# JensUweUlrich/Taxor

Hardware: AMD Instinct MI355X
Metric: Mbp/s classified (taxor search) vs GTDB k22/s12 (higher is better)
Workload: dtype u8

## Files before the change

taxor_amd/csrc/api.hip:

```cpp
#include "../../include/taxor_gpu_tools.h"
#include "fastx_scan.h"
#include "hip_host.h"
#include "ixf_arith.h"
#include "ixf_layout.h"
#include "kernels.h"
#include "saved_batch.h"
#include "tuning.h"

#include <sys/mman.h>

#include <algorithm>
#include <atomic>
#include <cstdio>
#include <cstring>
#include <mutex>
#include <string>
#include <thread>
#include <vector>

using namespace taxor;

namespace {

thread_local std::string g_err;
// ... 38 lines not shown
    std::mutex plane_mu;
    void *build_ctx = nullptr;
    void (*build_ctx_free)(void *) = nullptr;
    uint32_t n_passes = 0;
    std::vector<uint32_t> pass_of_ixf;
    std::vector<uint64_t> pass_data_bytes;
    uint64_t root_data_bytes = 0;
    uint32_t *d_binfo_full = nullptr;
    uint8_t *d_resident = nullptr;
    int cur_pass = -1;
    int up_group = -1;
    std::thread up_thread;
    int up_rc = 0;
    std::string up_err;
    std::vector<uint8_t> up_select;
    const uint8_t *upload_select = nullptr;
    double upload_wait_s = 0;
    std::mutex searchers_mu;
    std::vector<taxor_gpu_searcher *> searchers;
};

static void root_plane_invalidate(taxor_gpu_index *idx)
{
    std::lock_guard<std::mutex> lk(idx->plane_mu);
    idx->plane_valid = false;
}

static const uint8_t *root_plane_ensure(taxor_gpu_index *idx, hipStream_t st)
{
    if (!idx->plane_stride) return nullptr;
    std::lock_guard<std::mutex> lk(idx->plane_mu);
    if (idx->plane_valid) return idx->d_plane;
    if (!idx->d_plane && hipMalloc((void **)&idx->d_plane, idx->rows[0] * (uint64_t)idx->plane_stride) != hipSuccess) {
        (void)hipGetLastError();
        idx->d_plane = nullptr;
        idx->plane_stride = 0;
        return nullptr;
    }
    launch_build_plane(idx->h_ixf[0].data, idx->rows[0], idx->h_ixf[0].stride, idx->d_plane, idx->plane_stride, st);
    if (hipGetLastError() != hipSuccess || hipStreamSynchronize(st) != hipSuccess) return nullptr;
    idx->plane_valid = true;
    return idx->d_plane;
}

struct SubBatch {
    uint32_t first, n;
    uint32_t n_long = 0;
    uint64_t slots;
    uint64_t a_begin, a_end;
};

struct taxor_gpu_searcher {
    taxor_gpu_index *idx = nullptr;
    taxor_gpu_search_params prm{};
    std::vector<uint32_t> h_rlen, h_nh_sub;
    std::vector<uint64_t> lay_poff, lay_hoff, lay_aoff;
    std::vector<uint32_t> lay_hcap, lay_order;
    std::vector<uint64_t> h_thr_sub;
    bool thr_precomputed = false;
    std::vector<uint64_t> thr_memo;
    hipStream_t st = nullptr;
    hipStream_t st_sync = nullptr;
    hipStream_t st_sync2 = nullptr;
    hipEvent_t ev_wave = nullptr;
    hipStream_t st_copy = nullptr;
    std::vector<hipEvent_t> ev_sync_done, ev_query_done, ev_pack_done, ev_copy_done;
    hipEvent_t ev_reset = nullptr;
    DeviceBuf<uint32_t> d_sync_cursor;
    Counters *d_ctr = nullptr;
    unsigned long long *d_prof = nullptr;
    Counters h_ctr{};
    int grid_query_small[MAX_LEVELS] = {};
    size_t lds_query_small[MAX_LEVELS] = {};
    int grid_wave = 0, grid_wave_overlap = 0;
    int grid_sync = 0, grid_sync_overlap = 0, grid_query = 0, grid_query_short = 0;
    uint32_t first_div = 1;
    bool auto_sub_reads = true;
    bool prune = true;
    bool group_always = false;
    bool split_always = false;
    bool force_tree_stall = false;
    bool small_path = true;
    bool screen = true;
    size_t lds_query = 0;

    struct HostSpan { uint64_t vbegin, len; const char *ptr; };
    std::vector<HostSpan> host_spans;
    uint64_t n_reads = 0, n_bases = 0, mean_read_len = 1u << 20;
    DeviceBuf<uint8_t> d_ascii;
    DeviceBuf<uint64_t> d_aoff, d_poff, d_hoff;
    DeviceBuf<uint32_t> d_packed, d_rlen, d_hcap, d_nh, d_order;
    DeviceBuf<uint64_t> d_thr;
    std::vector<SubBatch> subs;
    uint64_t max_slots = 0, max_read_slots = 0;
    uint32_t max_sub_reads = 0;
    uint64_t packed_word_count = 0, packed_in_bytes = 0;
    FastxScan *fx = nullptr;
    std::vector<uint64_t> fx_off;
    DeviceBuf<uint64_t> d_boff;
    DeviceBuf<uint8_t> d_rev;
    std::vector<uint64_t> nib_off, nib_boff;
    std::vector<uint8_t> nib_rev;
    std::vector<uint32_t> h_words;

    DeviceBuf<uint64_t> d_cand[2], d_hashes[2];
    DeviceBuf<uint2> d_q[2], d_qs;
    DeviceBuf<uint32_t> d_qhist;
    DeviceBuf<uint4> d_hits;
    DeviceBuf<uint32_t> d_read_hits, d_cursor, d_roff, d_biglist, d_gtab, d_scan;
    uint32_t q_cap = 0, hit_cap = 0, gtab_stride = 0;

    DeviceBuf<uint64_t> d_read_off;
    DeviceBuf<int64_t> d_out_ub;
    DeviceBuf<uint32_t> d_out_cnt, d_out_key;
    uint64_t tuple_cap = 0;
    bool ran = false, synced = false;

    std::vector<uint64_t> h_read_off, h_hash_off, h_hashes;
    std::vector<int64_t> h_ub;
    std::vector<uint32_t> h_cnt, h_nh;
    void *h_small = nullptr;
    void *h_small_in = nullptr;

    struct SmallLane {
        taxor_gpu_searcher *c = nullptr;
        hipEvent_t done = nullptr, copied = nullptr;
        DeviceBuf<uint8_t> d_in;
        void *h_in = nullptr;
        size_t h_in_cap = 0;
        void *h_bases = nullptr;
        size_t h_bases_cap = 0;
        void *h_out = nullptr, *d_out = nullptr;
        uint32_t out_reads = 0, out_tuples = 0;
        bool fresh = true;
        bool q_dirty = false;
    };
    struct SmallPiece { uint32_t lane; uint64_t first, n; };
    std::vector<SmallLane> lanes;
    std::vector<SmallPiece> small_pieces;
    const char *small_bases = nullptr;
    const uint64_t *small_offsets = nullptr;
    bool lane_mode = false;
    bool st_borrowed = false;
    bool small_active = false, small_done = false;
    size_t small_harvested = 0;
    uint64_t small_tbase = 0;
    bool dev_results_stale = false;
    bool keep_keys = false;
    std::vector<uint32_t> h_key;

    bool capture = false;
    taxor_gpu_saved *cap_cur = nullptr;
    bool cap_done = false;
    DeviceBuf<uint64_t> d_cap_dense[2], d_cap_off;
    uint64_t *h_cap_pin[2] = {nullptr, nullptr};
    uint64_t *h_cap_total = nullptr;
    hipEvent_t ev_cap[2] = {nullptr, nullptr}, ev_cap_gather[2] = {nullptr, nullptr};
    hipStream_t st_cap = nullptr;
    const taxor_gpu_saved *replay = nullptr;
    bool from_saved = false;

    std::vector<hipEvent_t> ev;
    size_t ev_used = 0;
    std::vector<std::pair<size_t, int>> ev_spans;
    taxor_gpu_run_stats stats{};
};
// ... 753 lines not shown
    if (out) {
        const uint8_t *p = root_plane_ensure(idx, nullptr);
        if (!p) return TAXOR_OK;
        if (len != idx->rows[0] * (uint64_t)idx->plane_stride) return fail(TAXOR_E_ARG, "root_plane: the buffer does not match the plane");
        HIP_TRY(hipMemcpy(out, p, len, hipMemcpyDeviceToHost));
    }
    *rows = idx->rows[0];
    *plane_stride = idx->plane_stride;
    return TAXOR_OK;
}

extern "C" int taxor_gpu_index_download_ixf(const taxor_gpu_index *idx, uint64_t ixf, uint8_t *data, uint64_t len)
{
    if (!idx || ixf >= idx->h_ixf.size() || !data || len != idx->rows[ixf] * idx->h_ixf[ixf].stride)
        return fail(TAXOR_E_ARG, "download_ixf: bad arguments");
    HIP_TRY(hipSetDevice(idx->device));
    HIP_TRY(hipMemcpy(data, idx->h_ixf[ixf].data, len, hipMemcpyDeviceToHost));
    return TAXOR_OK;
}

static int searcher_create_impl(taxor_gpu_index *idx, const taxor_gpu_search_params *prm, taxor_gpu_searcher **out, hipStream_t lane_stream);

extern "C" int taxor_gpu_searcher_create(taxor_gpu_index *idx, const taxor_gpu_search_params *prm,
                                         taxor_gpu_searcher **out)
{
    return searcher_create_impl(idx, prm, out, nullptr);
}

static int searcher_create_impl(taxor_gpu_index *idx, const taxor_gpu_search_params *prm, taxor_gpu_searcher **out, hipStream_t lane_stream)
{
    if (!idx || !prm || !out) return fail(TAXOR_E_ARG, "searcher_create: null argument");
    const bool by_ratio = prm->model == TAXOR_THR_PERCENTAGE || prm->model == TAXOR_THR_SYNCMER;
    if (by_ratio && (!(prm->ratio >= 0.0) || !(prm->ratio <= 1.0)))
        return fail(TAXOR_E_ARG, "searcher_create: threshold ratio %g outside [0,1] (error rate / k outside the model?)", prm->ratio);
    if (prm->model > TAXOR_THR_FRACMINHASH) return fail(TAXOR_E_ARG, "searcher_create: unknown threshold model %u", prm->model);
    if (!by_ratio && (!(prm->error_rate > 0.0) || !(prm->error_rate < 1.0)))
        return fail(TAXOR_E_ARG, "searcher_create: the k-mer / FracMinHash threshold models need an error rate in (0,1), got %g", prm->error_rate);
    if (prm->model == TAXOR_THR_SYNCMER && idx->w_min > 0)
        return fail(TAXOR_E_ARG, "searcher_create: syncmer threshold model on an index built without syncmers");
    HIP_TRY(hipSetDevice(idx->device));
    auto s = new taxor_gpu_searcher();
    s->idx = idx;
    s->prm = *prm;
    s->auto_sub_reads = s->prm.sub_batch_reads == 0;
    if (s->prm.sub_batch_reads == 0) s->prm.sub_batch_reads = 32768;
    if (s->prm.sub_batch_bases == 0) s->prm.sub_batch_bases = 1ull << 29;
    if (s->prm.sub_batch_reads > (1u << 20)) s->prm.sub_batch_reads = 1u << 20;
    hipError_t e = hipSuccess;
    if (lane_stream) {
        s->st = lane_stream;
        s->st_borrowed = s->lane_mode = true;
    } else {
        e = hipStreamCreateWithFlags(&s->st, hipStreamNonBlocking);
        if (e == hipSuccess) e = hipStreamCreateWithFlags(&s->st_sync, hipStreamNonBlocking);
    }
    if (e == hipSuccess) e = hipEventCreateWithFlags(&s->ev_wave, hipEventDisableTiming);
    if (e == hipSuccess) e = hipEventCreateWithFlags(&s->ev_reset, hipEventDisableTiming);
    if (e == hipSuccess) e = hipMalloc((void **)&s->d_ctr, sizeof(Counters));
    if (e != hipSuccess) {
        delete s;
        return fail(TAXOR_E_HIP, "searcher_create: %s", hipGetErrorString(e));
    }
    s->lds_query = query_lds_bytes(idx->max_stride);
    if (s->lds_query > 160 * 1024) {
        taxor_gpu_searcher_destroy(s);
        return fail(TAXOR_E_ARG, "searcher_create: an IXF with %u-byte rows does not fit the LDS tally", idx->max_stride);
    }
    s->grid_sync = syncmers_grid(idx->device);
    if (const char *e = tune_env("TAXOR_PROFILE_PHASES")) {
        if (atoi(e) != 0 && (hipMalloc((void **)&s->d_prof, 16 * sizeof(unsigned long long)) != hipSuccess ||
                             hipMemset(s->d_prof, 0, 16 * sizeof(unsigned long long)) != hipSuccess)) {
            taxor_gpu_searcher_destroy(s);
            return fail(TAXOR_E_HIP, "searcher_create: profile buffer");
        }
    }
    s->prune = !(prm->flags & TAXOR_SEARCH_NO_PRUNE);
    s->group_always = (prm->flags & TAXOR_SEARCH_GROUP_ALWAYS) != 0;
    s->split_always = (prm->flags & TAXOR_SEARCH_SPLIT_ALWAYS) != 0;
    s->force_tree_stall = (prm->flags & TAXOR_SEARCH_FORCE_TREE_STALL) != 0;
    s->small_path = !(prm->flags & TAXOR_SEARCH_NO_SMALL_PATH);
    s->screen = !(prm->flags & TAXOR_SEARCH_NO_SCREEN);
    if (const char *e = tune_env("TAXOR_QUERY_PRUNE")) s->prune = atoi(e) != 0;
    if (const char *e = tune_env("TAXOR_QUERY_SCREEN")) s->screen = s->screen && atoi(e) != 0;
    if (const char *e = tune_env("TAXOR_FIRST_DIV")) { const int v = atoi(e); if (v >= 1 && v <= 64) s->first_div = (uint32_t)v; }
    if (const char *e = tune_env("TAXOR_SUB_READS")) { const long v = atol(e); if (v >= 1 && v <= (1 << 20)) { s->prm.sub_batch_reads = (uint32_t)v; s->auto_sub_reads = false; } }
    {
        hipDeviceProp_t p;
        int per = 2;
        if (const char *e = tune_env("TAXOR_SYNC_BPC_OVERLAP")) { const int v = atoi(e); if (v >= 1 && v <= 8) per = v; }
        s->grid_sync_overlap = hipGetDeviceProperties(&p, idx->device) == hipSuccess ? p.multiProcessorCount * per : s->grid_sync;
        if (s->grid_sync_overlap > s->grid_sync) s->grid_sync_overlap = s->grid_sync;
    }
    s->grid_wave = syncmers_wave_grid(idx->device, 8);
    {
        int per = 2;
        if (const char *e = tune_env("TAXOR_SYNC_BPC_OVERLAP")) { const int v = atoi(e); if (v >= 1 && v <= 8) per = v; }
        s->grid_wave_overlap = syncmers_wave_grid(idx->device, per);
    }
    s->grid_query = query_grid(idx->device, s->lds_query, 3);
    s->grid_query_short = query_grid(idx->device, s->lds_query, 4);
    {
        static const bool small_off = [] { const char *e = tune_env("TAXOR_QUERY_SMALL"); return e && atoi(e) == 0; }();
        for (uint32_t l = 0; l < idx->depth && l < (uint32_t)MAX_LEVELS && !small_off; ++l) {
            static const uint32_t max_stride_small = [] { const char *e = tune_env("TAXOR_QUERY_SMALL_MAXSTRIDE"); return e ? (uint32_t)atoi(e) : 512u; }();
            if (idx->lvl_max_stride[l] == 0 || idx->lvl_max_stride[l] > max_stride_small) continue;
            s->lds_query_small[l] = query_lds_bytes(idx->lvl_max_stride[l], true);
            s->grid_query_small[l] = query_grid_small(idx->device, s->lds_query_small[l]);
        }
    }
    s->keep_keys = idx->n_passes > 0;
    if (!lane_stream) {
        std::lock_guard<std::mutex> lk(idx->searchers_mu);
        idx->searchers.push_back(s);
    }
    *out = s;
    return TAXOR_OK;
}

static void capture_release(taxor_gpu_searcher *s)
{
    delete s->cap_cur;
    s->cap_cur = nullptr;
    s->cap_done = false;
    s->d_cap_off.release();
    if (s->st_cap) { (void)hipStreamSynchronize(s->st_cap); (void)hipStreamDestroy(s->st_cap); s->st_cap = nullptr; }
    for (int i = 0; i < 2; ++i) {
        s->d_cap_dense[i].release();
        if (s->ev_cap_gather[i]) (void)hipEventDestroy(s->ev_cap_gather[i]);
        s->ev_cap_gather[i] = nullptr;
        if (s->h_cap_pin[i]) (void)hipHostFree(s->h_cap_pin[i]);
        if (s->ev_cap[i]) (void)hipEventDestroy(s->ev_cap[i]);
        s->h_cap_pin[i] = nullptr;
        s->ev_cap[i] = nullptr;
    }
    if (s->h_cap_total) (void)hipHostFree(s->h_cap_total);
    s->h_cap_total = nullptr;
}

extern "C" void taxor_gpu_searcher_destroy(taxor_gpu_searcher *s)
{
    if (!s) return;
    {
        std::lock_guard<std::mutex> lk(s->idx->searchers_mu);
        auto &v = s->idx->searchers;
        v.erase(std::remove(v.begin(), v.end(), s), v.end());
    }
    (void)hipSetDevice(s->idx->device);
    for (auto &L : s->lanes) {
        if (L.c) { (void)hipStreamSynchronize(L.c->st); taxor_gpu_searcher_destroy(L.c); }
        if (L.done) (void)hipEventDestroy(L.done);
        if (L.copied) (void)hipEventDestroy(L.copied);
        L.d_in.release();
        if (L.h_in) (void)hipHostFree(L.h_in);
        if (L.h_bases) (void)hipHostFree(L.h_bases);
        if (L.h_out) (void)hipHostFree(L.h_out);
    }
    s->lanes.clear();
    capture_release(s);
    if (s->st_copy) (void)hipStreamSynchronize(s->st_copy);
    if (s->st_sync2) (void)hipStreamSynchronize(s->st_sync2);
    if (s->st_sync) (void)hipStreamSynchronize(s->st_sync);
    if (s->st) (void)hipStreamSynchronize(s->st);
    s->d_ascii.release(); s->d_aoff.release(); s->d_poff.release(); s->d_hoff.release();
    s->d_packed.release(); s->d_rlen.release(); s->d_hcap.release(); s->d_nh.release(); s->d_thr.release();
    s->d_order.release(); s->d_boff.release(); s->d_rev.release();
    if (s->fx) fastx_scan_destroy(s->fx);
// ... 229 lines not shown
    q.hashes = d_hashes;
    q.hoff = d_hoff;
    q.nh = d_nh;
    q.thr = d_thr;
    q.hits = s->d_hits.p;
    q.read_hits = s->d_read_hits.p;
    q.counts_out = d_counts_out;
    q.ctr = s->d_ctr;
    q.q_cap = s->q_cap;
    q.hit_cap = s->hit_cap;
    q.map_words = query_map_words(idx->max_stride);
    q.max_stride = idx->max_stride;
    q.prune = (d_counts_out == nullptr && s->prune) ? 1u : 0u;
    q.prof = s->d_prof;
    static const uint32_t stages_env = [] { const char *e = tune_env("TAXOR_QUERY_STAGES"); const int v = e ? atoi(e) : 0; return v >= 1 && v <= 64 ? (uint32_t)v : 0u; }();
    q.sparse_stages = stages_env;
    static const float margin_env = [] { const char *e = tune_env("TAXOR_QUERY_MARGIN"); const double v = e ? atof(e) : 0.0; return v > 0.0 && v < 64.0 ? (float)v : 0.f; }();
    q.prune_margin = margin_env;
    static const uint32_t tally_env = [] { const char *e = tune_env("TAXOR_QUERY_TALLY"); return e ? (uint32_t)atoi(e) & 3u : 0u; }();
    q.tally_mode = tally_env;
    static const uint32_t sort_env = [] { const char *e = tune_env("TAXOR_QUERY_SORT_UNITS"); return e ? (uint32_t)(atoi(e) != 0) : 0u; }();
    q.sort_units = sort_env;
    static const uint32_t dense_stride_env = [] { const char *e = tune_env("TAXOR_QUERY_DENSE_STRIDE"); return e ? (uint32_t)atoi(e) : 0u; }();
    q.dense_max_stride = dense_stride_env;
    if (root_parts == 0) root_parts = s->split_always ? idx->root_pmax : 1u;
    if (d_counts_out || only_ixf >= 0 || root_parts > idx->root_pmax || idx->root_pmax % root_parts != 0) root_parts = 1;
    q.parts = root_parts;
    for (uint32_t j = 0; j <= root_parts; ++j) q.part_cut[j] = idx->root_cut[j * (idx->root_pmax / root_parts)];
    q.part_cut[root_parts] = idx->root_cut[idx->root_pmax];
    if (tree) {
        q.level = 0;
        q.q_in = nullptr;
        q.q_out = s->d_q[0].p;
        q.n_level0 = n_reads;
        q.order0 = d_order;
        q.cursor_chunk = 1;
        q.xcd_slices = 0;
        const char *pe = tune_env("TAXOR_TREE_POLLS");
        q.tree_polls = s->force_tree_stall ? 0u : pe ? (uint32_t)std::max(0, atoi(pe)) : (1u << 22);
        const uint64_t items0 = (uint64_t)n_reads * root_parts;
        static const int grid_env = [] { const char *e = tune_env("TAXOR_TREE_GRID"); return e ? atoi(e) : 0; }();
        static const int unroll_env = [] { const char *e = tune_env("TAXOR_TREE_UNROLL"); return e ? atoi(e) : 0; }();
        const uint64_t grid_cap = grid_env > 0 ? (uint64_t)grid_env : (uint64_t)s->grid_query_short / 2;
        const int grid = (int)std::min<uint64_t>(grid_cap, std::max<uint64_t>(items0, 2ull * n_reads) + 64);
        launch_query_tree(q, grid, s->lds_query, s->st, unroll_env == 2 ? 2 : 4);
        s->stats.query_launches++;
        HIP_TRY(hipGetLastError());
        return 0;
    }
    const uint32_t levels = only_ixf >= 0 ? 1u : idx->depth;
    static const bool group_queue = [] { const char *e = tune_env("TAXOR_QUERY_GROUP"); return !e || atoi(e) != 0; }();
    for (uint32_t lvl = 0; lvl < levels; ++lvl) {
        q.level = lvl;
        q.q_in = (lvl == 0 && only_ixf < 0) ? nullptr : s->d_q[lvl & 1].p;
        const char *gm = tune_env("TAXOR_QUERY_GROUP_MIN");
        const uint32_t group_min = gm ? (uint32_t)atoi(gm) : (s->group_always ? 0u : 4096u);
        q.xcd_slices = 0;
        if (lvl >= 1 && only_ixf < 0 && group_queue && n_reads >= group_min) {
            static const uint32_t xcd_env = [] { const char *e = tune_env("TAXOR_QUERY_XCD"); const int v = e ? atoi(e) : 8;
                                                 return (v == 1 || v == 8) ? 8u : (v == 2 || v == 4) ? (uint32_t)v : 0u; }();
            q.xcd_slices = xcd_env;
            launch_queue_group_by_ixf(s->d_q[lvl & 1].p, s->d_ctr, lvl, s->q_cap, s->d_qhist.p, (uint32_t)idx->h_ixf.size(), s->d_qs.p, s->st);
            q.q_in = s->d_qs.p;
        }
        q.q_out = s->d_q[(lvl + 1) & 1].p;
        q.n_level0 = n_reads;
        q.order0 = d_order;
        static const uint32_t chunk_env = [] { const char *e = tune_env("TAXOR_QUERY_CHUNK"); return e ? (uint32_t)atoi(e) : 0u; }();
        q.cursor_chunk = chunk_env ? chunk_env : (lvl >= 1 ? 4u : (s->mean_read_len < 1500 ? 8u : (s->mean_read_len < 3000 ? 4u : 1u)));
        size_t slot;
        if (ev_begin(s, 16 + (int)std::min(lvl, 7u), &slot)) return TAXOR_E_HIP;
        static const int bpc_l1 = [] { const char *e = tune_env("TAXOR_QUERY_BPC_L1"); return e ? atoi(e) : 4; }();
        const uint64_t items0 = (uint64_t)n_reads * root_parts;
        const bool wide_grid = s->mean_read_len < 6000 || (lvl >= 1 && bpc_l1 >= 4) ||
                               (lvl == 0 && items0 > (uint64_t)s->grid_query && items0 <= (uint64_t)s->grid_query_short);
        const bool root_streams = idx->rows[0] * (uint64_t)idx->h_ixf[0].stride > (16ull << 30);
        const bool small = !d_counts_out && only_ixf < 0 && lvl < (uint32_t)MAX_LEVELS && s->grid_query_small[lvl] > 0 &&
                           s->mean_read_len < 2600 && !s->d_prof;
        q.plane = nullptr;
        q.plane_stride = 0;
        if (lvl == 0 && !small && s->screen && q.prune && !s->lane_mode && !s->d_prof && only_ixf < 0 && root_parts == 1) {
            q.plane = root_plane_ensure(s->idx, s->st);
            q.plane_stride = q.plane ? idx->plane_stride : 0;
        }
        if (small) {
            QueryArgs qs = q;
            qs.max_stride = idx->lvl_max_stride[lvl];
            qs.map_words = query_map_words(idx->lvl_max_stride[lvl]);
            qs.cursor_chunk = chunk_env ? chunk_env : 4;
            launch_query_level(qs, s->grid_query_small[lvl], s->lds_query_small[lvl], s->st, true, root_streams);
        } else
            launch_query_level(q, wide_grid ? s->grid_query_short : s->grid_query, s->lds_query, s->st, false, root_streams);
        if (ev_end(s, slot)) return TAXOR_E_HIP;
        s->stats.query_launches++;
    }
    HIP_TRY(hipGetLastError());
    if (d_counts_out || !finalize) return 0;
    FinalizeArgs f{};
    f.hits = s->d_hits.p;
    f.read_hits = s->d_read_hits.p;
    f.cursor = s->d_cursor.p;
    f.roff = s->d_roff.p;
    f.biglist = s->d_biglist.p;
    f.block_sums = s->d_scan.p;
    f.dfs_key = idx->d_dfs_key;
    f.ubin = idx->d_ubin;
    f.read_off = d_read_off;
    f.out_ub = s->d_out_ub.p;
    f.out_cnt = s->d_out_cnt.p;
    f.out_key = s->d_out_key.p;
    f.ctr = s->d_ctr;
    f.n_reads = n_reads;
    f.tuple_cap = s->tuple_cap;
    f.hit_cap = s->hit_cap;
    f.is_last = is_last;
    size_t slot;
    if (ev_begin(s, 2, &slot)) return TAXOR_E_HIP;
    launch_finalize(f, s->st);
    if (ev_end(s, slot)) return TAXOR_E_HIP;
    HIP_TRY(hipGetLastError());
    return 0;
}

int reset_sub_counters(taxor_gpu_searcher *s, bool whole)
{
    const size_t n = whole ? sizeof(Counters) : offsetof(Counters, tuple_total);
    if (whole) HIP_TRY(hipMemsetAsync(s->d_ctr, 0, n, s->st));
    else HIP_TRY(hipMemsetAsync(reinterpret_cast<uint8_t *>(s->d_ctr) + sizeof(uint32_t), 0, n - sizeof(uint32_t), s->st));
    return 0;
}

int launch_syncmers_sub(taxor_gpu_searcher *s, const SubBatch &sb, size_t sub_i, int buf, hipStream_t st,
                        bool overlapped = false, hipStream_t st_short = nullptr)
{
    if (!st_short) st_short = st;
    const taxor_gpu_index *idx = s->idx;
    SyncmerArgs a{};
    a.packed = s->d_packed.p;
    a.poff = s->d_poff.p + sb.first;
    a.rlen = s->d_rlen.p + sb.first;
    a.hoff = s->d_hoff.p + sb.first;
    a.hcap = s->d_hcap.p + sb.first;
    a.cand = s->d_cand[buf].p;
    a.hashes = s->d_hashes[buf].p;
    a.cursor = s->d_sync_cursor.p + 2 * sub_i;
    a.order = s->d_order.p ? s->d_order.p + sb.first : nullptr;
    a.nh = s->d_nh.p + sb.first;
    a.thr = s->d_thr.p + sb.first;
    a.ratio = s->prm.ratio;
    a.scaling_limit = idx->scaling > 1 ? (double)UINT64_MAX / (double)idx->scaling : 0.0;
    a.gtab = s->d_gtab.p;
    a.gtab_stride = s->gtab_stride;
    a.ctr = s->d_ctr;
    a.n_reads = sb.n;
    {
        static const uint32_t chunk_env = [] { const char *e = tune_env("TAXOR_SYNC_CHUNK"); return e ? (uint32_t)atoi(e) : 0u; }();
        a.chunk = chunk_env ? chunk_env : (s->mean_read_len < 2500 ? 8u : (s->mean_read_len < 6000 ? 4u : 1u));
    }
    a.k = idx->k;
    a.s = idx->s;
    a.t = idx->t;
    a.w_min = idx->w_min;
    a.thr_on_device = s->prm.model == TAXOR_THR_PERCENTAGE ? 1 : 0;
    a.prof = s->d_prof;
    size_t slot;
    if (ev_begin(s, 0, &slot, st)) return TAXOR_E_HIP;
// ... 1485 lines not shown
            s->h_hashes.insert(s->h_hashes.end(), tmp.begin() + hoff_h[r], tmp.begin() + hoff_h[r] + nh);
        }
    }
    *hash_off = s->h_hash_off.data();
    *hashes = s->h_hashes.data();
    return TAXOR_OK;
}

namespace {

int stage_hash_list(taxor_gpu_searcher *s, const uint64_t *hashes, uint64_t n, uint64_t threshold)
{
    if (n >= (1ull << 32)) return fail(TAXOR_E_ARG, "hash list too long");
    HIP_TRY(hipSetDevice(s->idx->device));
    s->ran = s->synced = false;
    s->small_active = false;
    s->replay = nullptr;
    s->from_saved = false;
    s->n_reads = 1;
    s->n_bases = 0;
    s->mean_read_len = 1u << 20;
    s->subs.clear();
    s->max_slots = n + 64;
    s->max_read_slots = 16;
    s->max_sub_reads = 1;
    if (reserve(s->d_hoff, 2) || reserve(s->d_nh, 2) || reserve(s->d_thr, 2)) return TAXOR_E_HIP;
    if (int rc = ensure_scratch(s)) return rc;
    const uint64_t zero = 0;
    const uint32_t nh = (uint32_t)n;
    if (n) HIP_TRY(hipMemcpy(s->d_hashes[0].p, hashes, n * 8, hipMemcpyHostToDevice));
    HIP_TRY(hipMemcpy(s->d_hoff.p, &zero, 8, hipMemcpyHostToDevice));
    HIP_TRY(hipMemcpy(s->d_nh.p, &nh, 4, hipMemcpyHostToDevice));
    HIP_TRY(hipMemcpy(s->d_thr.p, &threshold, 8, hipMemcpyHostToDevice));
    return 0;
}

}

extern "C" int taxor_gpu_ixf_bulk_count(taxor_gpu_searcher *s, uint64_t ixf, const uint64_t *hashes, uint64_t n,
                                        uint32_t *counts)
{
    if (!s || !counts || (n && !hashes)) return fail(TAXOR_E_ARG, "ixf_bulk_count: null argument");
    if (ixf >= s->idx->h_ixf.size()) return fail(TAXOR_E_ARG, "ixf_bulk_count: bad IXF id");
    if (int rc = stage_hash_list(s, hashes, n, ~0ull)) return rc;
    const uint32_t bins = s->idx->h_ixf[ixf].bins;
    uint32_t *d_counts = nullptr;
    HIP_TRY(hipMalloc((void **)&d_counts, (size_t)bins * 4));
    int rc = reset_sub_counters(s, true);
    const uint2 item = make_uint2(0u, (uint32_t)ixf);
    const uint32_t one = 1;
    hipError_t e = hipMemcpyAsync(s->d_q[0].p, &item, sizeof item, hipMemcpyHostToDevice, s->st);
    if (e == hipSuccess) e = hipMemcpyAsync(&s->d_ctr->q_n[0].v, &one, 4, hipMemcpyHostToDevice, s->st);
    if (e == hipSuccess) e = hipStreamSynchronize(s->st);
    if (e != hipSuccess) rc = fail(TAXOR_E_HIP, "ixf_bulk_count: %s", hipGetErrorString(e));
    s->ev_used = 0;
    s->ev_spans.clear();
    if (!rc) rc = run_query(s, s->d_hashes[0].p, s->d_hoff.p, s->d_nh.p, s->d_thr.p, 1, nullptr, 1, d_counts, (int)ixf);
    if (!rc) {
        e = hipStreamSynchronize(s->st);
        if (e == hipSuccess) e = hipMemcpy(counts, d_counts, (size_t)bins * 4, hipMemcpyDeviceToHost);
        if (e != hipSuccess) rc = fail(TAXOR_E_HIP, "ixf_bulk_count: %s", hipGetErrorString(e));
    }
    (void)hipFree(d_counts);
    return rc;
}

extern "C" int taxor_gpu_bulk_contains(taxor_gpu_searcher *s, const uint64_t *hashes, uint64_t n, uint64_t threshold,
                                       taxor_gpu_results *out)
{
    if (!s || !out || (n && !hashes)) return fail(TAXOR_E_ARG, "bulk_contains: null argument");
    if (int rc = stage_hash_list(s, hashes, n, threshold)) return rc;
    for (int attempt = 0; attempt < 40; ++attempt) {
        if (int rc = ensure_scratch(s)) return rc;
        if (reset_sub_counters(s, true)) return TAXOR_E_HIP;
        s->ev_used = 0;
        s->ev_spans.clear();
        if (int rc = run_query(s, s->d_hashes[0].p, s->d_hoff.p, s->d_nh.p, s->d_thr.p, 1, s->d_read_off.p, 1, nullptr, -1))
            return rc;
        bool rerun;
        if (int rc = check_flags(s, &rerun)) return rc;
        if (!rerun) {
            s->ran = s->synced = true;
            s->stats.screen_plane_loads = s->h_ctr.plane_loads;
            return taxor_gpu_batch_fetch(s, out);
        }
    }
    return fail(TAXOR_E_INTERNAL, "bulk_contains: buffers kept overflowing");
}
```

taxor_amd/csrc/kernels.h:

```cpp
#pragma once
#include <hip/hip_runtime.h>
#include <stdint.h>

namespace taxor {

struct IxfDesc {
    const uint8_t *data;
    uint64_t seed;
    uint32_t seg_len;
    uint32_t bins;
    uint32_t stride;
    uint32_t units;
    uint32_t bin_base;
    uint32_t arith;
};

static constexpr uint32_t BINFO_MERGED = 0x80000000u;
static constexpr uint32_t BINFO_END = 0x40000000u;

enum : uint32_t {
    FLAG_ALPHABET = 1u,
    FLAG_CAND_OVERFLOW = 2u,
    FLAG_QUEUE_OVERFLOW = 4u,
    FLAG_HITS_OVERFLOW = 8u,
// ... 8 lines not shown
};
struct Counters {
    uint32_t flags;
    uint32_t reserved0;
    uint32_t n_big;
    uint32_t pad0[29];
    PaddedU32 n_hits;
    PaddedU32 q_n[16];
    PaddedU32 q_cursor[16];
    PaddedU32 q_xcur[16][8];
    alignas(128) unsigned long long tuple_total;
    unsigned long long n_hashes;
    alignas(128) unsigned long long query_bytes;
    unsigned long long n_work;
    unsigned long long touched_bytes;
    unsigned long long plane_loads;
    unsigned long long pad1[12];
    unsigned long long lvl_touched[8];
    unsigned long long lvl_rows[8];
    unsigned long long lvl_sparse[8];
};
static constexpr int MAX_LEVELS = 16;

static constexpr uint32_t SYNC_LDS_DEDUP_MAX = 66816;
static constexpr uint32_t SYNC_WAVE_CAND = 512;

struct SyncmerArgs {
    const uint32_t *packed;
    const uint64_t *poff;
    const uint32_t *rlen;
    const uint64_t *hoff;
    const uint32_t *hcap;
    uint64_t *cand;
    uint64_t *hashes;
    uint32_t *nh;
    uint64_t *thr;
    double ratio;
    double scaling_limit;
    uint32_t *gtab;
    uint32_t gtab_stride;
    Counters *ctr;
    uint32_t *cursor;
    const uint32_t *order;
    uint32_t n_reads;
    uint32_t chunk;
    int k, s, t;
    int w_min;
    int thr_on_device;
    unsigned long long *prof;
};

struct QueryArgs {
    const IxfDesc *ixf;
    const uint32_t *binfo;
    const uint64_t *hashes;
    const uint64_t *hoff;
    const uint32_t *nh;
    const uint64_t *thr;
    const uint2 *q_in;
    uint2 *q_out;
    uint4 *hits;
    uint32_t *read_hits;
    uint32_t *counts_out;
    Counters *ctr;
    uint32_t level;
    uint32_t n_level0;
    const uint32_t *order0;
    uint32_t q_cap, hit_cap;
    uint32_t map_words;
    uint32_t max_stride;
    uint32_t prune;
    uint32_t cursor_chunk;
    float prune_margin;
    uint32_t sparse_stages;
    uint32_t xcd_slices;
    uint32_t parts;
    uint16_t part_cut[10];
    uint32_t tree_polls;
    uint32_t sort_units;
    uint32_t dense_max_stride;
    uint32_t tally_mode;
    const uint8_t *plane;
    uint32_t plane_stride;
    unsigned long long *prof;
};

struct FinalizeArgs {
    const uint4 *hits;
    uint32_t *read_hits;
    uint32_t *cursor;
    uint32_t *roff;
    uint32_t *biglist;
    uint32_t *block_sums;
    const uint32_t *dfs_key;
    const int64_t *ubin;
    uint64_t *read_off;
    int64_t *out_ub;
    uint32_t *out_cnt;
    uint32_t *out_key;
    Counters *ctr;
    uint32_t n_reads;
    uint64_t tuple_cap;
    uint32_t hit_cap;
    int is_last;
};

static constexpr uint32_t SMALL_FIN_MAX = 4096;
struct SmallFinalizeArgs {
    const uint4 *hits;
    uint32_t *read_hits;
    const uint32_t *dfs_key;
    const int64_t *ubin;
    const uint32_t *nh;
    uint32_t *key, *cnt;
    int64_t *ub;
    Counters *ctr;
    uint32_t *sync_cursor;
    uint32_t n_reads, tuple_cap, hit_cap;
    uint64_t *h_read_off;
    uint32_t *h_nh;
    int64_t *h_ub;
    uint32_t *h_cnt;
    uint64_t *h_status;
};
void launch_finalize_small(const SmallFinalizeArgs &a, hipStream_t st);

void launch_pack_dna4(const uint8_t *ascii, const uint64_t *aoff, const uint64_t *poff, uint32_t *packed,
                      uint32_t n_reads, Counters *ctr, hipStream_t st, int max_grid = 0);
void launch_pack_nibbles(const uint8_t *seq4, const uint64_t *boff, const uint32_t *rlen, const uint8_t *rev, const uint64_t *poff,
                         uint32_t *packed, uint32_t n_reads, Counters *ctr, hipStream_t st, int max_grid = 0);
void launch_syncmers(const SyncmerArgs &a, int grid, hipStream_t st);
void launch_syncmers_wave(const SyncmerArgs &a, int grid, hipStream_t st);
int syncmers_wave_grid(int device, int want_per_cu);
bool syncmers_wave_applies(int k, int s);
int syncmers_grid(int device);
void launch_query_level(const QueryArgs &a, int grid, size_t lds_bytes, hipStream_t st, bool small = false, bool root_streams = true);
void launch_query_tree(const QueryArgs &a, int grid, size_t lds_bytes, hipStream_t st, int unroll = 2);
int query_grid(int device, size_t lds_bytes, int want_per_cu);
int query_grid_small(int device, size_t lds_bytes);
size_t query_lds_bytes(uint32_t max_stride, bool small = false);
uint32_t query_map_words(uint32_t max_stride);
void launch_finalize(const FinalizeArgs &a, hipStream_t st);
void launch_queue_group_by_ixf(const uint2 *q, const Counters *ctr, uint32_t lvl, uint32_t q_cap, uint32_t *hist, uint32_t n_ixf,
                               uint2 *out, hipStream_t st);
void launch_fill_random(uint8_t *data, uint64_t n_bytes, uint64_t seed, hipStream_t st);
uint64_t launch_gather_sparse(const uint8_t *data, uint64_t rows, uint32_t stride, uint32_t bins, uint64_t want_loads, uint64_t seed,
                              uint32_t *sink, bool nt, hipStream_t st);
uint64_t launch_gather_ceiling(const uint8_t *data, uint64_t rows, uint32_t stride, uint32_t bins, uint64_t want_bytes,
                               uint64_t seed, uint32_t *sink, bool nt, hipStream_t st, uint32_t n_ixf = 1, uint64_t spacing = 0);
void launch_scatter_column(uint8_t *data, uint64_t stride, uint64_t bin, const uint8_t *col, uint64_t rows,
                           hipStream_t st);
inline uint32_t plane_stride_of(uint32_t stride) { return (stride / 4u + 127u) & ~127u; }
void launch_build_plane(const uint8_t *data, uint64_t rows, uint32_t stride, uint8_t *plane, uint32_t plane_stride, hipStream_t st);

void launch_binfo_pass(const uint32_t *full, const uint8_t *resident, uint32_t *binfo, uint32_t n_bins, uint32_t n_ixf, hipStream_t st);

struct MergeList {
    const uint64_t *read_off;
    const int64_t *ub;
    const uint32_t *cnt, *key;
};
struct MergeArgs {
    const MergeList *lists;
    uint32_t n_lists, n_reads;
    uint32_t *s_key, *s_cnt;
    int64_t *s_ub;
// ... 18 lines not shown
```

taxor_amd/csrc/kernels.hip:

```cpp
#include "kernels.h"
#include "device_prims.h"
#include "ixf_arith.h"
#include "tuning.h"

#include <algorithm>
#include <cstdlib>

namespace taxor {

static constexpr int BLK = 256;

__global__ __launch_bounds__(BLK) void k_pack_dna4(const uint8_t *__restrict__ ascii,
                                                   const uint64_t *__restrict__ aoff,
                                                   const uint64_t *__restrict__ poff,
                                                   uint32_t *__restrict__ packed, uint32_t n_reads,
                                                   Counters *ctr)
{
    __shared__ uint8_t sLut[256];
    sLut[threadIdx.x] = (uint8_t)dna4_code((uint8_t)threadIdx.x);
    __syncthreads();
    for (uint32_t r = blockIdx.x; r < n_reads; r += gridDim.x) {
        const uint64_t a0 = aoff[r];
        const uint32_t len = (uint32_t)(aoff[r + 1] - a0);
        const uint32_t nw = ((len + 15u) >> 4);
// ... 1172 lines not shown
                    m.thr = a.thr[m.r];
                    m.hoff = a.hoff[m.r];
                    m.n = a.nh[m.r];
                    sItems[0] = m;
                }
                item = item0 = 0u;
                item_end = 1u;
                __syncthreads();
            } else
            if (a.xcd_slices) {
                if (tid == 0) {
                    const uint32_t S = a.xcd_slices;
                    const uint32_t per = (n_items + S - 1u) / S;
                    uint32_t got = n_items, got_end = n_items;
                    for (uint32_t k = 0; k < S; ++k) {
                        const uint32_t sl = (((blockIdx.x & 7u) * S >> 3) + k) & (S - 1u);
                        const uint32_t lo = min(sl * per, n_items), hi = min(lo + per, n_items);
                        if (lo >= hi) continue;
                        const uint32_t i = atomicAdd(&a.ctr->q_xcur[min(lvl, 15u)][sl].v, chunk);
                        if (i < hi - lo) { got = lo + i; got_end = hi; break; }
                    }
                    sScal[0] = got;
                    sScal[7] = got_end;
                }
                __syncthreads();
                item = item0 = sScal[0];
                item_end = min(item + chunk, sScal[7]);
                if (item >= n_items) break;
            } else {
                if (tid == 0) sScal[0] = atomicAdd(&a.ctr->q_cursor[lvl].v, chunk);
                __syncthreads();
                item = item0 = sScal[0];
                item_end = min(item + chunk, n_items);
                if (item >= n_items) break;
            }
            if (!TREE && tid < item_end - item) {
                uint32_t r_, v_, part = 0;
                if (a.q_in) { const uint2 it = a.q_in[item + tid]; r_ = it.x; v_ = it.y; }
                else {
                    uint32_t ri = item + tid;
                    if (n_parts > 1u) { part = ri / a.n_level0; ri -= part * a.n_level0; }
                    r_ = a.order0 ? a.order0[ri] : ri;
                    v_ = 0;
                }
                ItemMeta m;
                m.D = a.ixf[v_];
                if (n_parts > 1u) {
                    const uint32_t u0 = a.part_cut[part], u1 = a.part_cut[part + 1u];
                    m.D.data += (size_t)u0 * 16u;
                    m.D.bin_base += u0 * 16u;
                    m.D.bins = min(m.D.bins, u1 * 16u) - u0 * 16u;
                    m.D.units = u1 - u0;
                }
                m.thr = a.thr[r_];
                m.hoff = a.hoff[r_];
                m.r = r_;
                m.n = a.nh[r_];
                sItems[tid] = m;
            }
            __syncthreads();
        }
        PMARK(0)
        const IxfDesc D = sItems[item - item0].D;
        const uint32_t r = sItems[item - item0].r, n = sItems[item - item0].n;
        const uint64_t thr = sItems[item - item0].thr;
        const uint64_t *__restrict__ hp = a.hashes + sItems[item - item0].hoff;
        const uint32_t stride = D.stride;
        const uint32_t *__restrict__ bi = a.binfo + D.bin_base;
        const uint32_t nb_round = (D.bins + 63u) & ~63u;

        const bool info_cached = info_of == D.bin_base && !(a.tally_mode & 2u);
        const bool info_regs = nb_round <= 4u * BS;
        uint32_t infoReg[4] = {0u, 0u, 0u, 0u};
        if (info_regs && !info_cached) {
#pragma unroll
            for (int j = 0; j < 4; ++j) {
                const uint32_t b = tid + (uint32_t)j * BS;
                if (b < D.bins) infoReg[j] = bi[b];
            }
        }
        for (uint32_t i = tid; i < stride; i += BS) sC[i] = 0;
        for (uint32_t i = tid; i < a.map_words; i += BS) { sMap[i] = 0; sCandMap[i] = 0; }
        if (tid == 0) { sScal[1] = 0; sScal[6] = 0; }

        uint32_t dense_end = n;
        if (a.prune && thr > 0 && stride > a.dense_max_stride) {
            const float mu = thr < (uint64_t)n ? (float)((uint64_t)n - thr) * (1.0f / 256.0f) : 0.0f;
            const uint32_t margin = (uint32_t)(mu + 4.0f * sqrtf(mu) + (a.prune_margin > 0.f ? a.prune_margin : 3.5f));
            dense_end = (thr >= (uint64_t)n + margin) ? 0u : min(n, (uint32_t)((uint64_t)n + margin - thr));
        }
        uint64_t touched = 0, rows_read = 0, sparse_loads = 0;
        uint32_t d2 = 0;
        if constexpr (SCREEN) {
            if (n >= (uint32_t)SCR_MIN_HASHES && dense_end > 0u && dense_end < n && thr <= (uint64_t)n) {
                const float x = (float)((uint64_t)n - thr);
                const float m2 = 4.0f * sqrtf(0.1875f * (x * (1.0f / 0.75f) + 16.0f)) + 2.0f;
                const float d = ceilf((x + m2) * (1.0f / 0.75f));
                if (d <= (float)n) d2 = max((uint32_t)d, 1u);
            }
        }
        const bool screen = SCREEN && d2 > 0u;

        const bool staged = n <= (uint32_t)QC;
        if (staged)
            for (uint32_t i = tid; i < n; i += BS) {
                const ixf_probe p = ixf_probe_key_arith(hp[i], D.seed, D.seg_len, D.arith);
                sProbe[i] = make_uint4(p.row[0], p.row[1], p.row[2], p.fp4);
            }
        if (info_cached) {
        } else if (info_regs) {
#pragma unroll
            for (int j = 0; j < 4; ++j) {
                const uint32_t b = tid + (uint32_t)j * BS;
                if (b < nb_round) sInfo[b] = infoReg[j];
            }
        } else {
            for (uint32_t b = tid; b < nb_round; b += BS) sInfo[b] = b < D.bins ? bi[b] : 0u;
        }
        info_of = D.bins ? D.bin_base : 0xFFFFFFFFu;
        __syncthreads();
        PMARK(1)
        if (screen) {
            query_screen_range<NT, BS, QC>(D, a.plane, a.plane_stride, hp, d2, sProbe, sC, staged);
            touched += (uint64_t)d2 * 3ull * a.plane_stride;
            st_plane += (unsigned long long)d2 * 3ull;
        } else {
            query_dense_range<NT, U, BS, QC>(D, hp, 0, dense_end, sProbe, sC, staged);
            touched += (uint64_t)dense_end * 3ull * (D.units * 16u);
            rows_read += (uint64_t)dense_end * 3ull;
        }
        __syncthreads();
        PMARK(2)

        bool cand_valid = false;
        if (dense_end < n) {
            uint32_t done = screen ? 0u : dense_end;
            uint32_t chunk = 0;
            bool first_eval = true;
            cand_valid = !a.counts_out && !(a.tally_mode & 1u);
            for (;;) {
                uint64_t rem = (screen && first_eval) ? n - d2 : n - done;
                const bool on_plane = screen && first_eval;
                if (!first_eval) {
                    for (uint32_t i = tid; i < a.map_words; i += BS) sMap[i] = 0;
                    if (tid == 0) sScal[1] = 0;
                    __syncthreads();
                }
                for (uint32_t b = tid; b < nb_round; b += BS) {
                    if (b < D.bins) {
                        const uint32_t info = sInfo[b];
                        const bool dead_on_plane = screen && !first_eval && !((sCandMap[b >> 9] >> ((b >> 4) & 31u)) & 1u);
                        if ((info & BINFO_END) && !dead_on_plane) {
                            int bb = (int)b;
                            uint64_t sum = sC[bb];
                            bool alive, cand;
                            if (info & BINFO_MERGED) {
                                cand = sum + rem >= thr;
                                alive = cand && (on_plane || sum < thr);
                            } else {
                                while (bb > 0 && (sInfo[bb - 1] >> 30) == 0u) sum += sC[--bb];
                                const uint64_t len = (uint64_t)b - (uint64_t)bb + 1u;
                                alive = cand = sum + rem * len >= thr;
                            }
                            if (first_eval && cand) {
                                for (uint32_t x = (uint32_t)bb >> 4; x <= (b >> 4); ++x) {
                                    const uint32_t bit = 1u << (x & 31u);
                                    if (!(atomicOr(&sCandMap[x >> 5], bit) & bit)) {
                                        const uint32_t k = atomicAdd(&sScal[6], 1u);
                                        if (k < (uint32_t)Q_MAXC) sCandUnits[k] = x;
                                    }
                                }
                            }
                            if (alive) {
                                for (uint32_t x = (uint32_t)bb >> 4; x <= (b >> 4); ++x) {
                                    const uint32_t bit = 1u << (x & 31u);
                                    if (!(atomicOr(&sMap[x >> 5], bit) & bit)) {
                                        const uint32_t k = atomicAdd(&sScal[1], 1u);
                                        if (k < (uint32_t)Q_MAXU) sUnits[k] = x;
                                    }
                                }
                            }
                        }
                    }
                }
                __syncthreads();
                if (a.sort_units && sScal[1] > 1u && sScal[1] <= (uint32_t)Q_MAXU) {
                    const uint32_t na = sScal[1];
                    uint32_t x = 0xFFFFFFFFu, rank = 0;
                    if (tid < na) x = sUnits[tid];
                    if (tid < 64u) {
                        for (uint32_t j = 0; j < na; ++j) rank += (__shfl(x, (int)j) < x) ? 1u : 0u;
                    }
                    __syncthreads();
                    if (tid < na) sUnits[rank] = x;
                    __syncthreads();
                }
                if (first_eval) { PMARK(3) }
                if (on_plane) {
                    for (uint32_t i = tid; i < stride; i += BS) sC[i] = 0;
                    rem = n;
                    __syncthreads();
                }
                const uint32_t n_alive = sScal[1];
                if (n_alive == 0) break;
                if (n_alive > (uint32_t)Q_MAXU) {
                    query_dense_range<NT, U, BS, QC>(D, hp, done, n, sProbe, sC, staged);
                    touched += rem * 3ull * (D.units * 16u);
                    rows_read += rem * 3ull;
                    break;
                }
                if (first_eval) {
                    const uint32_t want = a.sparse_stages ? a.sparse_stages : 3u;
                    const uint32_t stages = rem >= 128u * want ? want : max(1u, (uint32_t)(rem / 128u));
                    chunk = staged ? (uint32_t)((rem + stages - 1u) / stages) : min((uint32_t)Q_HT2, (uint32_t)QC);
                    first_eval = false;
                }
                const uint32_t nt = min(chunk, n - done);
                const uint4 *pr = sProbe + (staged ? done : 0u);
                if (!staged) {
                    for (uint32_t i = tid; i < nt; i += BS) {
                        const ixf_probe p = ixf_probe_key_arith(hp[done + i], D.seed, D.seg_len, D.arith);
                        sProbe[i] = make_uint4(p.row[0], p.row[1], p.row[2], p.fp4);
                    }
                    __syncthreads();
                }
                const uint32_t tasks = nt * n_alive;
                constexpr int SU = 4;
                for (uint32_t task0 = tid; task0 < tasks; task0 += BS * SU) {
                    uint4 r0[SU], r1[SU], r2[SU];
                    uint32_t xs[SU], fp4[SU];
#pragma unroll
                    for (int u = 0; u < SU; ++u) {
                        const uint32_t task = task0 + (uint32_t)u * BS;
                        xs[u] = 0xFFFFFFFFu;
                        r0[u] = r1[u] = r2[u] = make_uint4(0, 0, 0, 0);
                        fp4[u] = 0;
                        if (task < tasks) {
                            const uint32_t i = task / n_alive, j = task - i * n_alive;
                            xs[u] = sUnits[j];
                            const uint4 p = pr[i];
                            fp4[u] = p.w;
                            const uint8_t *base = D.data + (size_t)xs[u] * 16u;
                            r0[u] = ld16<NT>(base + (size_t)p.x * stride);
                            r1[u] = ld16<NT>(base + (size_t)p.y * stride);
                            r2[u] = ld16<NT>(base + (size_t)p.z * stride);
                        }
                    }
#pragma unroll
                    for (int u = 0; u < SU; ++u) {
                        if (xs[u] == 0xFFFFFFFFu) continue;
                        const uint32_t z[4] = {zero_bytes01(r0[u].x ^ r1[u].x ^ r2[u].x ^ fp4[u]), zero_bytes01(r0[u].y ^ r1[u].y ^ r2[u].y ^ fp4[u]),
                                               zero_bytes01(r0[u].z ^ r1[u].z ^ r2[u].z ^ fp4[u]), zero_bytes01(r0[u].w ^ r1[u].w ^ r2[u].w ^ fp4[u])};
#pragma unroll
                        for (int q = 0; q < 4; ++q) {
                            uint32_t m = z[q];
                            while (m) {
                                const int bit = __ffs((int)m) - 1;
                                m &= m - 1u;
                                atomicAdd(&sC[xs[u] * 16u + 4u * (uint32_t)q + ((uint32_t)bit >> 3)], 1u);
                            }
                        }
                    }
                }
                touched += (uint64_t)nt * (uint64_t)n_alive * 3ull * 64ull;
                rows_read += (uint64_t)nt * (uint64_t)n_alive * 3ull;
                sparse_loads += (uint64_t)nt * (uint64_t)n_alive * 3ull;
                done += nt;
                __syncthreads();
                if (done >= n) break;
            }
        }
        __syncthreads();
        PMARK(4)

        if (a.counts_out)
            for (uint32_t b = tid; b < D.bins; b += BS) a.counts_out[b] = sC[b];

        const uint32_t n_cand = sScal[6];
        const bool cand_tally = cand_valid && n_cand <= (uint32_t)Q_MAXC;
        const uint32_t t_end = cand_tally ? ((n_cand * 16u + 63u) & ~63u) : nb_round;
        for (uint32_t t = tid; t < t_end; t += BS) {
            bool push_child = false, push_hit = false;
            uint32_t sum = 0, info = 0;
            uint32_t b = t;
            if (cand_tally) b = t < n_cand * 16u ? sCandUnits[t >> 4] * 16u + (t & 15u) : 0xFFFFFFFFu;
            if (b < D.bins) {
                info = sInfo[b];
                if (info & BINFO_MERGED) {
                    sum = sC[b];
                    push_child = (uint64_t)sum >= thr && (info & 0x3FFFFFFFu) != 0u;
                } else if (info & BINFO_END) {
                    int bb = (int)b;
                    sum = sC[bb];
                    while (bb > 0 && (sInfo[bb - 1] >> 30) == 0u) sum += sC[--bb];
                    push_hit = (uint64_t)sum >= thr;
                }
            }
            const uint32_t qs = wave_append(push_child, &sScal[2]);
            if (push_child) {
                const uint2 rec = make_uint2(r, info & 0x3FFFFFFFu);
// ... 804 lines not shown
```

Baseline: 33910.

## Adaptively re-evaluate bin survival at predicted decision points in screened root query

Measured after the change: 33800. About the same (-0.3%).

```diff
diff --git a/taxor_amd/csrc/api.hip b/taxor_amd/csrc/api.hip
--- a/taxor_amd/csrc/api.hip
+++ b/taxor_amd/csrc/api.hip
@@ -144,6 +144,9 @@
     bool force_tree_stall = false;
     bool small_path = true;
     bool screen = true;
+    uint32_t recount = 1;
+    uint32_t recount_step = 0;
+    float recount_sigma = 0.f;
     size_t lds_query = 0;
 
     struct HostSpan { uint64_t vbegin, len; const char *ptr; };
@@ -1063,6 +1066,9 @@
     s->screen = !(prm->flags & TAXOR_SEARCH_NO_SCREEN);
     if (const char *e = tune_env("TAXOR_QUERY_PRUNE")) s->prune = atoi(e) != 0;
     if (const char *e = tune_env("TAXOR_QUERY_SCREEN")) s->screen = s->screen && atoi(e) != 0;
+    if (const char *e = tune_env("TAXOR_QUERY_RECOUNT")) s->recount = atoi(e) != 0 ? 1u : 0u;
+    if (const char *e = tune_env("TAXOR_QUERY_RECOUNT_STEP")) { const int v = atoi(e); if (v >= 1 && v <= 4096) s->recount_step = (uint32_t)v; }
+    if (const char *e = tune_env("TAXOR_QUERY_RECOUNT_SIGMA")) { const double v = atof(e); if (v > 0.0 && v < 64.0) s->recount_sigma = (float)v; }
     if (const char *e = tune_env("TAXOR_FIRST_DIV")) { const int v = atoi(e); if (v >= 1 && v <= 64) s->first_div = (uint32_t)v; }
     if (const char *e = tune_env("TAXOR_SUB_READS")) { const long v = atol(e); if (v >= 1 && v <= (1 << 20)) { s->prm.sub_batch_reads = (uint32_t)v; s->auto_sub_reads = false; } }
     {
@@ -1458,6 +1464,9 @@
         if (lvl == 0 && !small && s->screen && q.prune && !s->lane_mode && !s->d_prof && only_ixf < 0 && root_parts == 1) {
             q.plane = root_plane_ensure(s->idx, s->st);
             q.plane_stride = q.plane ? idx->plane_stride : 0;
+            q.recount = s->recount;
+            q.recount_step = s->recount_step;
+            q.recount_sigma = s->recount_sigma;
         }
         if (small) {
             QueryArgs qs = q;
@@ -3109,6 +3118,10 @@
         if (!rerun) {
             s->ran = s->synced = true;
             s->stats.screen_plane_loads = s->h_ctr.plane_loads;
+            for (int l = 0; l < 8; ++l) {
+                s->stats.level_row_reads[l] = s->h_ctr.lvl_rows[l];
+                s->stats.level_sparse_loads[l] = s->h_ctr.lvl_sparse[l];
+            }
             return taxor_gpu_batch_fetch(s, out);
         }
     }
diff --git a/taxor_amd/csrc/kernels.h b/taxor_amd/csrc/kernels.h
--- a/taxor_amd/csrc/kernels.h
+++ b/taxor_amd/csrc/kernels.h
@@ -114,6 +114,9 @@
     uint32_t tally_mode;
     const uint8_t *plane;
     uint32_t plane_stride;
+    uint32_t recount;
+    uint32_t recount_step;
+    float recount_sigma;
     unsigned long long *prof;
 };
 
diff --git a/taxor_amd/csrc/kernels.hip b/taxor_amd/csrc/kernels.hip
--- a/taxor_amd/csrc/kernels.hip
+++ b/taxor_amd/csrc/kernels.hip
@@ -1278,6 +1278,8 @@
         for (uint32_t i = tid; i < stride; i += BS) sC[i] = 0;
         for (uint32_t i = tid; i < a.map_words; i += BS) { sMap[i] = 0; sCandMap[i] = 0; }
         if (tid == 0) { sScal[1] = 0; sScal[6] = 0; }
+        if constexpr (SCREEN)
+            if (tid == 0) { sScal[9] = 0xFFFFFFFFu; sScal[10] = 0; }
 
         uint32_t dense_end = n;
         if (a.prune && thr > 0 && stride > a.dense_max_stride) {
@@ -1332,6 +1334,7 @@
         if (dense_end < n) {
             uint32_t done = screen ? 0u : dense_end;
             uint32_t chunk = 0;
+            uint32_t rc_step = 0;
             bool first_eval = true;
             cand_valid = !a.counts_out && !(a.tally_mode & 1u);
             for (;;) {
@@ -1340,9 +1343,14 @@
                 if (!first_eval) {
                     for (uint32_t i = tid; i < a.map_words; i += BS) sMap[i] = 0;
                     if (tid == 0) sScal[1] = 0;
+                    if constexpr (SCREEN)
+                        if (tid == 0) { sScal[9] = 0xFFFFFFFFu; sScal[10] = 0; }
                     __syncthreads();
                 }
-                for (uint32_t b = tid; b < nb_round; b += BS) {
+                const bool cand_walk = SCREEN && rc_step != 0u && sScal[6] <= (uint32_t)Q_MAXC;
+                const uint32_t e_end = cand_walk ? sScal[6] * 16u : nb_round;
+                for (uint32_t t = tid; t < e_end; t += BS) {
+                    const uint32_t b = cand_walk ? sCandUnits[t >> 4] * 16u + (t & 15u) : t;
                     if (b < D.bins) {
                         const uint32_t info = sInfo[b];
                         const bool dead_on_plane = screen && !first_eval && !((sCandMap[b >> 9] >> ((b >> 4) & 31u)) & 1u);
@@ -1353,6 +1361,26 @@
                             if (info & BINFO_MERGED) {
                                 cand = sum + rem >= thr;
                                 alive = cand && (on_plane || sum < thr);
+                                if constexpr (SCREEN) {
+                                    if (alive) sScal[10] = 1u;
+                                    if (alive && a.recount) {
+                                        const float fn = (float)n, ft = (float)thr, ks = a.recount_sigma > 0.f ? a.recount_sigma : 2.0f;
+                                        float pt = 0.0f;
+                                        if (on_plane) {
+                                            const float fd = (float)d2;
+                                            const float rho = fminf(fmaxf(((float)sum / fd - 0.25f) * (1.0f / 0.75f), 0.0f), 1.0f);
+                                            const float sig = ks * sqrtf(0.1875f * fd * (1.0f - rho)) * (1.0f / 0.75f);
+                                            pt = rho * fn >= ft ? (ft + sig) / rho : (fn - ft + sig) / fmaxf(1.0f - rho, 1e-3f);
+                                        } else if (sum * 4u >= (uint64_t)done) {
+                                            const float fdn = (float)done, fs = (float)sum;
+                                            const float rho = fminf(fs / fdn, 1.0f);
+                                            const float need = ft - fs, miss = fmaxf((fn - ft) - (fdn - fs), 0.0f);
+                                            pt = fdn + (rho * fn >= ft ? (need + ks * sqrtf(need * (1.0f - rho))) / rho
+                                                                       : (miss + ks * sqrtf(miss * rho)) / fmaxf(1.0f - rho, 1e-3f));
+                                        }
+                                        if (pt > 0.0f) atomicMin(&sScal[9], (uint32_t)fminf(pt + 1.0f, fn));
+                                    }
+                                }
                             } else {
                                 while (bb > 0 && (sInfo[bb - 1] >> 30) == 0u) sum += sC[--bb];
                                 const uint64_t len = (uint64_t)b - (uint64_t)bb + 1u;
@@ -1410,8 +1438,21 @@
                     const uint32_t stages = rem >= 128u * want ? want : max(1u, (uint32_t)(rem / 128u));
                     chunk = staged ? (uint32_t)((rem + stages - 1u) / stages) : min((uint32_t)Q_HT2, (uint32_t)QC);
                     first_eval = false;
-                }
-                const uint32_t nt = min(chunk, n - done);
+                    if constexpr (SCREEN) {
+                        if (screen && a.recount && sScal[9] != 0xFFFFFFFFu)
+                            rc_step = a.recount_step ? a.recount_step : 64u;
+                    }
+                }
+                uint32_t nt = min(chunk, n - done);
+                if constexpr (SCREEN) {
+                    if (rc_step) {
+                        const uint32_t pt = sScal[9];
+                        uint32_t to = pt != 0xFFFFFFFFu ? max(pt, done + rc_step / 2u) : (sScal[10] ? done + rc_step : n);
+                        if (to >= n || n - to < rc_step / 2u) to = n;
+                        nt = to - done;
+                        if (!staged) nt = min(nt, chunk);
+                    }
+                }
                 const uint4 *pr = sProbe + (staged ? done : 0u);
                 if (!staged) {
                     for (uint32_t i = tid; i < nt; i += BS) {
```
